# dscripka/openWakeWord

Measured on AMD Instinct MI355X. Metric: real-time audio frames/sec (80 ms frame, 3 wakewords), whole job; real-time streams = value/12.5, higher is better.
Workload: dtype f32 as 3xf16 split MFMA, fp32 accumulate; 1 GPU; 131072 concurrent 16 kHz streams per GPU x 3 heads (alexa,hey_mycroft,hey_jarvis), 80 ms frames, BASELINE configs[3] per-GPU shard; streams_per_gpu=131072, frame_samples=1280, collective=none, gather=none, rccl_ranks=0, pcm_distribution=Gaussian, RMS 3000, pcm=resident in HBM, kernels=mfma_rr_f16x3, graph=False, vad=off, weights=synthetic seed 1234, step_blocks=1

## Files before the change

### openwakeword_amd/csrc/owwhip.hip

```cpp
#include <hip/hip_runtime.h>

#include <algorithm>
#include <cmath>
#include <cstdio>
#include <cstdlib>
#include <cstring>
#include <ctime>
#include <exception>
#include <mutex>
#include <new>
#include <unordered_map>
#include <dlfcn.h>
#include <string>
#include <vector>

#include "owwhip.h"
#include "owwhip_pack.h"
#include "owwhip_ingest.h"
#include "owwhip_mem.h"
#include "owwhip_masked_host.h"
#include "owwhip_bank_host.h"
#include "owwhip_verifier_host.h"
#include "owwhip_state_host.h"
#include "owwhip_kernels.h"
// ... 186 lines not shown
        bool busy = false;
    } slot[2];
    struct EventBuf {
        DevBuf<oww_event> d_rec; DevBuf<int> d_count; DevBuf<float> d_snap;
        DevBuf<int16_t> d_asnap;
        PinnedBuf<oww_event> h_rec; PinnedBuf<int> h_count;
    };
    int evt_cap = 0, evt_rows = 0;
    DevBuf<float> d_evt_thr; float evt_bank_thr = 0.5f;
    DevBuf<int> d_evblock; int evt_blocks = 0;
    EventBuf evt_sync, evt_slot[2];
    const EventBuf* evt_cur = nullptr;
    int aud_ring = 0, aud_evt = 0;
    DevBuf<int16_t> d_aring;
    DevBuf<uint32_t> d_acount;
    DevBuf<int16_t> d_aout; DevBuf<int> d_aids; DevBuf<uint32_t> d_acnt;

    uint64_t n_submit = 0, n_collect = 0;
    DevBuf<float> d_featinit, d_dbg;
    DevBuf<long long> d_prof;
    int prof_block = -1;
    DevBuf<uint32_t> d_nfeat, d_npred, d_nvad;
    DevBuf<float> d_vadring, d_vadin; float vad_threshold = 0.f;
    bool vad = false;
    const float *d_vad_hann = nullptr, *d_vad_encw = nullptr, *d_vad_encb = nullptr, *d_vad_lstmw = nullptr, *d_vad_lstmb = nullptr, *d_vad_wd = nullptr;
    float vad_bd = 0.f, vad_gain = 50.f;
    DevBuf<float> d_vadx, d_vadhc, d_vadlast;
    DevBuf<int16_t> d_tail, d_pcm;
    DevBuf<int16_t> d_long;
    DevBuf<float> d_callmax;
    PinnedBuf<int> h_range;
    int* d_range = nullptr;
    DevBuf<char> d_rs;
    std::vector<float> rs_taps;
    struct Ingest {
        bool ready = false, mixed = false;
        owi::Table tab;
        DevBuf<float> d_taps;
        DevBuf<int16_t> d_hist;
        DevBuf<int16_t> d_out;
        DevBuf<char> d_in;
        DevBuf<uint8_t> d_on;
        DevBuf<IngestClass> d_table;
        DevBuf<uint32_t> d_cls;
        DevBuf<int> d_newcls;
    } ing;
    DevBuf<uint8_t> d_on;
    DevBuf<int> d_lists; PinnedBuf<int> h_lists[2]; owm::Event lists_ev[2]; unsigned lists_turn = 0;
    int k_last = 1;
    float hx_absmax[20] = {};
    std::vector<int16_t> cal_user;
    int small_wgs = kSmallLaunchWgs, small_wgs_heads = kSmallLaunchWgs;
    int resident_b = -1, resident_b_wgs = kResidentBWgs;
    float hx_selftest_err = 0.f, hx_selftest_ref = 0.f, hx_selftest_score_err = 0.f;
    bool fuse = false;
    DevBuf<float> d_verw, d_verb, d_verthr; DevBuf<int> d_verT;
    int ver_stride = 0, n_verifiers = 0;
    std::vector<int> ver_T;
    bool post_in_heads = false;
    DevBuf<float> d_save;
    DevBuf<int> d_ids;
    DevBuf<int> d_patience;
    DevBuf<float> d_threshold;
    int debounce_frames = 0;
    void* comm = nullptr; int comm_rank = 0, comm_world = 1;
    bool timing = false;
    std::vector<EventRec> ev;
    size_t ev_used = 0;
    double t_ms[OWW_N_KERNEL_CLASSES] = {};
    int64_t t_n[OWW_N_KERNEL_CLASSES] = {};
    bool want_graph = false;
    hipGraph_t graph = nullptr;
    hipGraphExec_t graph_exec = nullptr;
    struct BankHead {
        bool live = false;
        int T = 0, hidden = 0, has_ln = 0, ht = 4, patience = 0;
        float threshold = NAN;
        DevBuf<float> d_img;
        size_t w1_bytes = 0;
        owh::BankHeadDev dev{};
    };
    int bank_K = 0, bank_cap = 0;
    std::vector<BankHead> bank;
    std::vector<int> bank_sub;
    DevBuf<int> d_bank_sub, d_bank_idx;
    DevBuf<float> d_bank_raw, d_bank_scores, d_bank_ring;
    DevBuf<uint32_t> d_bank_npred;
    DevBuf<owh::BankHeadDev> d_bank_heads; DevBuf<int> d_bank_pat; DevBuf<float> d_bank_thr;
    DevBuf<owh::BankTile> d_bank_tiles; DevBuf<int> d_bank_entries;
    owb::Route bank_rt;
    int vpool_cap = 0;
    int vpool_stride = 0;
    std::vector<int> vpool_T;
    DevBuf<float> d_vpool_w, d_vpool_b;
    std::vector<int> vasg_fix, vasg_bank;
    std::vector<float> vthr_fix, vthr_bank;
    long long vasg_n = 0;
    std::vector<float> ver_thr;
    DevBuf<SvEntry> d_svlist; int sv_n = 0;
    DevBuf<unsigned long long> d_sv_eval;
    bool st_ready = false;
    std::vector<ows::FlatSection> st_flat;
    std::vector<ows::GroupSection> st_group;
    bool st_levels[4] = {};
    DevBuf<ows::FlatSection> d_st_flat;
    uint32_t st_record_words = 0, st_flat_quads = 0;
// ... 72 lines not shown
        p.xout = h->d_xA; p.dbg = dbg ? h->d_dbg : nullptr; p.dbg_stride = DBG_FLOATS;
        Timed t(h, 1);
        hipLaunchKernelGGL(stageA_kernel<MFMA>, dim3(n_active), dim3(CfgA::NT), CfgA::LDS_BYTES, st, p);
    }
    auto fill = [&](StageParams& p, const float* xin, float* xout, int first_layer, int sb, int sd) {
        p.xin = xin; p.xout = xout; p.hist_b = h->d_state[sb]; p.hist_d = h->d_state[sd];
        for (int i = 0; i < 4; ++i) {
            p.w[i] = h->d_conv[first_layer + i]; p.scale[i] = h->d_scale[first_layer + i];
            p.shift[i] = h->d_shift[first_layer + i]; p.dbg_off[i] = dbg_off[first_layer + i];
        }
        p.dbg = dbg ? h->d_dbg : nullptr; p.dbg_stride = DBG_FLOATS;
        p.prof = h->d_prof ? h->d_prof + (first_layer / 4) * 256 : nullptr;
        p.prof_block = h->prof_block;
    };
    {
        StageParams p{}; fill(p, h->d_xA, h->d_xB, 3, 2, 3);
        Timed t(h, 2);
        hipLaunchKernelGGL((stage_kernel<CfgB, MFMA, false>), dim3((n_active + CfgB::B - 1) / CfgB::B), dim3(CfgB::NT), CfgB::LDS_BYTES, st, p);
    }
    {
        StageParams p{}; fill(p, h->d_xB, h->d_xC, 7, 4, 5);
        Timed t(h, 3);
        hipLaunchKernelGGL((stage_kernel<CfgC, MFMA, false>), dim3((n_active + CfgC::B - 1) / CfgC::B), dim3(CfgC::NT), CfgC::LDS_BYTES, st, p);
    }
    {
        StageParams p{}; fill(p, h->d_xC, h->d_xD, 11, 6, 7);
        Timed t(h, 4);
        hipLaunchKernelGGL((stage_kernel<CfgD, MFMA, false>), dim3((n_active + CfgD::B - 1) / CfgD::B), dim3(CfgD::NT), CfgD::LDS_BYTES, st, p);
    }
    {
        StageParams p{}; fill(p, h->d_xD, nullptr, 15, 8, 9);
        p.hist19 = h->d_state[10]; p.w19 = h->d_conv[19]; p.feat = h->d_feat; p.emb = h->d_emb; p.nfeat = h->d_nfeat; p.TR = h->TR;
        p.dbg_off[4] = dbg_off[19];
        Timed t(h, 5);
        hipLaunchKernelGGL((stage_kernel<CfgE, MFMA, true>), dim3((n_active + CfgE::B - 1) / CfgE::B), dim3(CfgE::NT), CfgE::LDS_BYTES, st, p);
    }
    HIPCHK(hipGetLastError());
    return 0;
}

template <class CR, class CH, int WG, bool LAST, bool DBG, bool HX>
void launch_rstage(oww_ctx* h, const owr::RStageParams& p, int cls) {
    hipStream_t st = h->stream;
    Timed t(h, cls);
    const int nwg = (p.n_groups + WG - 1) / WG;
    if constexpr (HX && !DBG && std::is_same<CH, owh::HB>::value) {
        const bool resident = p.glist == nullptr && p.n_groups > 0 && (h->resident_b < 0 ? p.n_groups >= kResidentBMinGroups : h->resident_b != 0);
        if (resident) {
            const int grid = std::max(1, std::min(h->resident_b_wgs, (p.n_groups + owh::RES_B_WG - 1) / owh::RES_B_WG));
            hipLaunchKernelGGL((owh::hstage_kernel<CH, LAST, false, owh::RES_B_WG, 1>), dim3(grid), dim3(64 * owh::RES_B_WG), owh::RES_B_LDS_BYTES, st, p);
            return;
        }
    }
    if (HX && !DBG && nwg <= h->small_wgs) hipLaunchKernelGGL((owh::hstage_kernel<CH, LAST, false, WG, 3>), dim3(nwg), dim3(64 * WG), 0, st, p);
    else if (HX) hipLaunchKernelGGL((owh::hstage_kernel<CH, LAST, DBG, WG>), dim3(nwg), dim3(64 * WG), 0, st, p);
    else hipLaunchKernelGGL((owr::rstage_kernel<CR, LAST, DBG>), dim3((p.n_groups + 3) / 4), dim3(256), 0, st, p);
}

template <bool DBG, bool HX>
int run_cnn_rr(oww_ctx* h, const StepArgs& a, int n_active, int mel_stride, int mel_off) {
    using namespace owr;
    hipStream_t st = h->stream;
    int off = 0, dbg_off[20];
    for (int l = 0; l < 20; ++l) { dbg_off[l] = off; off += kLayerOut[l][0] * kLayerOut[l][1] * kLayerOut[l][2]; }
    {
        RAParams p{};
        p.mel = a.mel ? a.mel : h->d_mel; p.mel_stride = mel_stride; p.mel_off = mel_off;
        p.hist_mel = h->d_state[0]; p.hist2 = h->d_state[1];
        p.w0 = h->d_conv[0]; p.w1 = h->d_conv[1]; p.w2 = h->d_conv[2];
        for (int i = 0; i < 3; ++i) { p.scale[i] = h->d_scale[i]; p.shift[i] = h->d_shift[i]; p.dbg_off[i] = dbg_off[i]; }
        p.xout = h->d_xA; p.n_streams = n_active; p.S = h->Spad;
        p.dbg = DBG ? h->d_dbg : nullptr; p.dbg_stride = DBG_FLOATS;
        for (int i = 0; i < 3; ++i) { p.clampv[i] = -0.4f * ldexpf(1.f, h->hx_e[i]); p.dbg_mul[i] = ldexpf(1.f, -h->hx_e[i]); }
        p.xmul = ldexpf(1.f, h->hx_xexp[0]);
        p.range_flag = HX ? h->d_range : nullptr;
        p.stream_on = a.on;
        const int grid = std::min((n_active + 3) / 4, 768);
        Timed t(h, 1);
        if (HX && a.fused_pcm) {
            owf::MelAParams q{};
            q.a = p; q.a.mel = nullptr; q.a.n_streams = h->S;
            q.pcm = a.fused_pcm; q.tail = h->d_tail; q.nfeat = h->d_nfeat; q.hann = h->d_hann; q.mel_start = h->d_mstart; q.mel_taps = h->d_taps; q.mel_off = h->d_meloff; q.mel_dst = h->d_meldst;
            q.mel_out = h->cfg.debug_layers ? h->d_mel : nullptr;
            const int per_cu = std::max(1, std::min(12 / owf::FA_WG, 163840 / owf::FA_LDS_BYTES));
            const int g2 = std::max(1, std::min((q.a.n_streams + owf::FA_WG - 1) / owf::FA_WG, 256 * per_cu));
            hipLaunchKernelGGL(owf::hmelA_kernel<DBG>, dim3(g2), dim3(64 * owf::FA_WG), owf::FA_LDS_BYTES, st, q);
        }
        else if (HX) hipLaunchKernelGGL(owh::hstageA_kernel<DBG>, dim3(std::min((n_active + 3) / 4, 256 * OWH_WPS_A)), dim3(256), 0, st, p);
        else hipLaunchKernelGGL(rstageA_kernel<DBG>, dim3(grid), dim3(256), 0, st, p);
    }
    auto fill = [&](const float* xin, float* xout, int first_layer, int sb, int sd, int spt) {
        RStageParams p{};
        p.xin = xin; p.xout = xout; p.hist_b = h->d_state[sb]; p.hist_d = h->d_state[sd];
        for (int i = 0; i < 4; ++i) {
            p.w[i] = h->d_conv[first_layer + i]; p.scale[i] = h->d_scale[first_layer + i];
            p.shift[i] = h->d_shift[first_layer + i]; p.dbg_off[i] = dbg_off[first_layer + i];
            p.clampv[i] = -0.4f * ldexpf(1.f, h->hx_e[first_layer + i]); p.dbg_mul[i] = ldexpf(1.f, -h->hx_e[first_layer + i]);
        }
        p.dbg_mul[4] = ldexpf(1.f, -h->hx_e[19]);
        p.xmul = ldexpf(1.f, h->hx_xexp[first_layer / 4 + 1]);
        p.emb_mul = ldexpf(1.f, -h->hx_e[19]);
        p.n_groups = (n_active + spt - 1) / spt; p.S = h->Spad;
        p.dbg = DBG ? h->d_dbg : nullptr; p.dbg_stride = DBG_FLOATS;
        p.range_flag = HX ? h->d_range : nullptr;
        p.stream_on = a.on;
        if (HX && a.lists) {
// ... 1370 lines not shown
    if (absmax) memcpy(absmax, h->hx_absmax, sizeof h->hx_absmax);
    if (exps) { for (int l = 0; l < 20; ++l) exps[l] = h->hx_e[l]; exps[20] = h->hx_efeat; }
    if (n_probe_streams) *n_probe_streams = CAL_NP + (int32_t)(h->cal_user.size() / ((size_t)CAL_T * OWW_CHUNK));
    if (selftest) { selftest[0] = h->hx_selftest_err; selftest[1] = h->hx_selftest_ref; selftest[2] = h->hx_selftest_score_err; }
    return OWW_OK;
    OWW_GUARD_END
}

int oww_n_labels(const oww_ctx* h) { return h ? h->NL : 0; }

int oww_commit(oww_ctx* h) {
    OWW_GUARD_BEGIN
    if (!h) return fail(OWW_EINVAL, "null handle");
    if (h->committed) return fail(OWW_ESTATE, "already committed");
    if (h->mel_blob.empty() || h->emb_blob.empty()) return fail(OWW_ESTATE, "mel and embedding weights must be loaded before commit");
    HIPCHK(hipSetDevice(h->cfg.device));
    h->feature_ring = h->cfg.feature_ring;
    if (int rc = build_nets(*h, h->NL, h->TR, h->generic_hmax)) return rc;
    if (h->evt_rows > h->TR)
        return fail(OWW_EINVAL, "oww_events_configure: feature_rows = %d exceeds the handle's feature ring (%d rows)", h->evt_rows, h->TR);
    if (int rc = owa::commit_check(h->aud_evt, h->evt_cap)) return rc;
    CommitClock clk(h->hx ? "f16-split" : "family");
    HxCalib cal;
    if (h->hx) {
        if (int rc = calibrate_hx(h, cal)) return rc;
        h->probe_emb = cal.ref_emb; h->probe_nb = cal.nb;
        clk.lap("calibration (total)");
        if (getenv("OWW_DEBUG_CALIB"))
            for (int l = 0; l < 20; ++l) fprintf(stderr, "calib layer %2d: max|a| %-12.5g e_in %4d e_out %4d\n", l, h->hx_absmax[l], h->hx_ein[l], h->hx_e[l]);
    }
    HostBuf hb;
    WeightOff off;
    HeadGroups hg;
    h->no_wide_heads = getenv("OWW_NO_WIDE_HEADS") != nullptr;
    if (int rc = pack_mel_tables(*h, hb, off)) return rc;
    if (int rc = pack_cnn(*h, hb, off)) return rc;
    pack_net_arrays(*h, hb, off);
    if (int rc = pack_head_groups(*h, hg, hb, off)) return rc;
    h->groups.clear();
    for (const HeadGroup& g : hg.groups) h->groups.push_back(FastGroup{g});
    h->generic_nets = hg.generic_nets; h->rnn_nets = hg.rnn_nets;
    h->vad = !h->vad_blob.empty();
    if (int rc = pack_vad(*h, hb, off, h->vad_gain, h->vad_bd)) return rc;
    clk.lap("weight packing (host)");
    if (int rc = bind_weights(h, hb, off)) return rc;
    if (int rc = alloc_range_flag(h)) return rc;
    clk.lap("weight upload");
    if (int rc = alloc_state(h)) return rc;
    h->fuse = h->hx && !getenv("OWW_NO_FUSE");
    if (const char* e = getenv("OWW_SMALL_WGS")) h->small_wgs = atoi(e);
    if (const char* e = getenv("OWW_SMALL_WGS_HEADS")) h->small_wgs_heads = atoi(e);
    if (const char* e = getenv("OWW_RESIDENT_B")) h->resident_b = strcmp(e, "auto") == 0 ? -1 : (atoi(e) != 0 ? 1 : 0);
    if (const char* e = getenv("OWW_RESIDENT_B_WGS")) h->resident_b_wgs = std::max(1, atoi(e));
    if (const char* e = getenv("OWW_GENERIC_SPW")) { const int v = atoi(e); h->generic_spw = v == 4 || v == 16 ? v : 0; }
    h->post_in_heads = h->fuse && h->groups.size() == 1 && h->groups[0].ht == 4 && h->generic_nets.empty() && h->rnn_nets.empty() && h->NL > 0;
    if (int rc = set_kernel_lds(h)) return rc;
    clk.lap("state allocation");
    if (int rc = derive_reset_state(h, cal, clk)) return rc;
    if (h->bank_K > 0) if (int rc = alloc_bank(h)) return rc;
    if (h->vpool_cap > 0) if (int rc = alloc_verifiers(h)) return rc;
    if (audio_on(h)) if (int rc = alloc_audio(h)) return rc;
    if (events_on(h)) if (int rc = alloc_events(h)) return rc;
    h->committed = true;
    return OWW_OK;
    OWW_GUARD_END
}

int oww_reset(oww_ctx* h, const int32_t* stream_ids, int32_t n, const float* init_features) {
    OWW_GUARD_BEGIN
    if (!h || !h->committed) return fail(OWW_ESTATE, "oww_reset: handle not committed");
    HIPCHK(hipSetDevice(h->cfg.device));
    const float* d_init = nullptr;
    if (init_features) {
        HIPCHK(copy_async(h->d_featinit, init_features, (size_t)h->TR * 96 * sizeof(float), hipMemcpyHostToDevice, h->stream));
        d_init = h->d_featinit;
    }
    if (!stream_ids) {
        if (int rc = do_reset(h, nullptr, h->Spad, d_init)) return rc;
    } else {
        if (n < 1) return OWW_OK;
        for (int i = 0; i < n; ++i)
            if (stream_ids[i] < 0 || stream_ids[i] >= h->S) return fail(OWW_EINVAL, "oww_reset: stream id %d out of range", stream_ids[i]);
        if (int rc = upload_ids(h, stream_ids, n)) return rc;
        if (int rc = do_reset(h, h->d_ids, n, d_init)) return rc;
    }
    if (h->ing.ready && h->ing.tab.Hpad_max) {
        hipLaunchKernelGGL(ingest_hist_reset_kernel, dim3(stream_ids ? n : h->S), dim3(64), 0, h->stream, h->ing.d_hist, h->ing.tab.Hpad_max,
                           stream_ids ? h->d_ids : nullptr, stream_ids ? n : h->S);
        HIPCHK(hipGetLastError());
    }
    if (audio_on(h)) if (int rc = audio_reset(h, stream_ids ? (const int*)h->d_ids : nullptr, n)) return rc;
    std::vector<int> slots;
    if (h->bank_K > 0) {
        if (!stream_ids) for (int i = 0; i < h->S * h->bank_K; ++i) slots.push_back(i);
        else for (int i = 0; i < n; ++i) for (int k = 0; k < h->bank_K; ++k) slots.push_back(stream_ids[i] * h->bank_K + k);
        if (int rc = bank_clear(h, slots)) return rc;
    }
    HIPCHK(hipStreamSynchronize(h->stream));
    return OWW_OK;
    OWW_GUARD_END
}

int oww_set_postproc(oww_ctx* h, const int32_t* patience, const float* threshold, int32_t debounce_frames) {
    OWW_GUARD_BEGIN
    if (!h || !h->committed) return fail(OWW_ESTATE, "oww_set_postproc: handle not committed");
    HIPCHK(hipSetDevice(h->cfg.device));
// ... 1574 lines not shown
```

### openwakeword_amd/csrc/owwhip_hx.h

```cpp
#pragma once
#include <type_traits>
#include <utility>
#include "owwhip_bank_host.h"
#include "owwhip_layout.h"
#include "owwhip_rr.h"

namespace owh {

using owr::f32x4;
typedef _Float16 f16x8 __attribute__((ext_vector_type(8)));

constexpr float WUNSCALE = 1.0f / 256.0f;

__device__ __forceinline__ float act1(float x, float cl) {
    return fmaxf(fmaxf(0.2f * x, x), cl);
}
template <bool ACT, bool HALF>
__device__ __forceinline__ f32x4 act_t(const f32x4 v, float cl) {
    if (!ACT) return HALF ? f32x4{v[0], v[1], 0.f, 0.f} : v;
    if (HALF) return f32x4{act1(v[0], cl), act1(v[1], cl), 0.f, 0.f};
    return f32x4{act1(v[0], cl), act1(v[1], cl), act1(v[2], cl), act1(v[3], cl)};
}
template <bool HALF>
__device__ __forceinline__ void pin_t(f32x4& v) {
// ... 337 lines not shown
                        const float l = dpp_shr_zero<SH>(accs[0][t][e]);
                        acc[t][e] = unpaired<F>(I[e] + ((MASKS && first) ? 0.f : l));
                    }
                }
            }
#pragma unroll
            for (int ks = 0; ks < KSI; ++ks) {
                f16x8 ah, al;
                if constexpr (AP) {
                    const int g = ti * KSI + ks;
                    const int ntap = ks + 1 < KSI ? tap : (ti == 0 ? 2 : 1), nks = ks + 1 < KSI ? ks + 1 : 0;
                    apipe_step(ap[g & 1], ap[(g + 1) & 1], cur, g + 1 < 3 * KSI ? (ntap * KSI + nks) * 2 : -1, lane);
                    ah = ap[g & 1].h; al = ap[g & 1].l;
                } else {
                    ah = lds_h(cur, (tap * KSI + ks) * 2 + 0, lane);
                    al = lds_h(cur, (tap * KSI + ks) * 2 + 1, lane);
                }
                if (REM2 && ks == KSI - 1) {
#pragma unroll
                    for (int t = 0; t < NT; ++t) acc[t] = OWH_MFMA(ah, in[t][ks].l, acc[t]);
#pragma unroll
                    for (int t = 0; t < NT; ++t) acc[t] = OWH_MFMA(al, in[t][ks].h, acc[t]);
                    continue;
                }
#pragma unroll
                for (int t = 0; t < NT; ++t) acc[t] = OWH_MFMA(ah, in[t][ks].h, acc[t]);
#pragma unroll
                for (int t = 0; t < NT; ++t) acc[t] = OWH_MFMA(ah, in[t][ks].l, acc[t]);
#pragma unroll
                for (int t = 0; t < NT; ++t) acc[t] = OWH_MFMA(al, in[t][ks].h, acc[t]);
            }
#pragma unroll
            for (int t = 0; t < NT; ++t) {
                if (ti < 2) accs[ti][t] = acc[t];
                else {
#pragma unroll
                    for (int e = 0; e < 4; ++e) {
                        if (HOUT && oct == NCTO - 1 && e >= 2) { res[t][e] = 0.f; continue; }
                        const float hh = dpp_shl_zero<SH>(accs[1][t][e]);
                        res[t][e] = acc[t][e] + ((MASKS && last) ? 0.f : hh);
                    }
                }
            }
        }
        if (oct == 0) {
#pragma unroll
            for (int t = 0; t < NT; ++t) nan_guard(bad, res[t][0]);
        }
#pragma unroll
        for (int t = 0; t < NT; ++t) {
            if (HOUT && oct == NCTO - 1) { out[t][oct] = act_t<BN, true>(res[t], cl); pin_t<true>(out[t][oct]); }
            else { out[t][oct] = act_t<BN, false>(res[t], cl); pin_t<false>(out[t][oct]); }
        }
        ring_end<NS, NBLK, NCTO, NEXT_NBLK, WG>(oct);
    }
}

template <int KSI, int NT, int F, int NPR>
__device__ __forceinline__ void merge_mel_rems(const Op (&in)[NT][KSI], Op (&M)[NT][(3 * NPR + 3) / 4]) {
    typedef unsigned u32x4 __attribute__((ext_vector_type(4)));
    static_assert(kInterleave || F == 16, "the operand shift relies on the zero fill at the stream edges");
    constexpr int SH = 16 / F, NMK = (3 * NPR + 3) / 4;
#pragma unroll
    for (int t = 0; t < NT; ++t) {
        const u32x4 sh = __builtin_bit_cast(u32x4, in[t][KSI - 1].h), sl = __builtin_bit_cast(u32x4, in[t][KSI - 1].l);
        unsigned h[NMK * 4], l[NMK * 4];
#pragma unroll
        for (int i = 0; i < NMK * 4; ++i) {
            const int tap = i / NPR, v = i % NPR;
            if (i >= 3 * NPR) { h[i] = 0u; l[i] = 0u; }
            else if (tap == 0) { h[i] = __builtin_amdgcn_update_dpp(0, sh[v], 0x110 + SH, 0xf, 0xf, true); l[i] = __builtin_amdgcn_update_dpp(0, sl[v], 0x110 + SH, 0xf, 0xf, true); }
            else if (tap == 2) { h[i] = __builtin_amdgcn_update_dpp(0, sh[v], 0x100 + SH, 0xf, 0xf, true); l[i] = __builtin_amdgcn_update_dpp(0, sl[v], 0x100 + SH, 0xf, 0xf, true); }
            else { h[i] = sh[v]; l[i] = sl[v]; }
        }
#pragma unroll
        for (int mk = 0; mk < NMK; ++mk) {
            M[t][mk].h = __builtin_bit_cast(f16x8, u32x4{h[4 * mk], h[4 * mk + 1], h[4 * mk + 2], h[4 * mk + 3]});
            M[t][mk].l = __builtin_bit_cast(f16x8, u32x4{l[4 * mk], l[4 * mk + 1], l[4 * mk + 2], l[4 * mk + 3]});
            pin_op(M[t][mk]);
        }
    }
}
template <int KSI, int NMK, int NCTO, int NT, int F, bool BN, int CH0, int NEXT_NBLK, int WG = OWH_WG, bool HOUT = false, int NS = 2, bool AP = false>
__device__ __forceinline__ void conv_mel_hxm(const Op (&in)[NT][KSI], const Op (&M)[NT][NMK], f32x4 (&out)[NT][NCTO], const WRing<NS>& ring,
                                             const float* __restrict__ w, const float* __restrict__ w_next,
                                             const float* __restrict__ init, float cl, int wave, int lane,
                                             lanemask_t& bad) {
    using namespace owr;
    const int j = lane >> 4;
    constexpr int SH = 16 / F, KSF = KSI - 1;
    constexpr int NBLK = (3 * KSF + NMK) * 2;
#pragma unroll
    for (int oct = 0; oct < NCTO; ++oct) {
        const float* cur = ring_begin<NS, CH0, NBLK, NCTO, NEXT_NBLK, WG>(ring, oct, w, w_next, wave, lane);
        f32x4 res[NT], accs[2][NT];
        APair ap[2];
        if constexpr (AP) ap[0] = apair_load(cur, 0, lane);
        int g = 0;
#pragma unroll
        for (int ti = 0; ti < 3; ++ti) {
            const int tap = ti == 0 ? 0 : (ti == 1 ? 2 : 1);
            f32x4 acc[NT];
            f32x4 I = {0.f, 0.f, 0.f, 0.f};
            if (ti == 2) I = acc_init(BN ? init : nullptr, oct, j);
#pragma unroll
            for (int t = 0; t < NT; ++t) {
// ... 264 lines not shown
#ifndef OWH_HIST_LDS
#define OWH_HIST_LDS 1
#endif
#ifndef OWH_HIST_LDS_C
#define OWH_HIST_LDS_C 0
#endif
#ifndef OWH_SPRIO_B
#define OWH_SPRIO_B 1111
#endif
#ifndef OWH_SPRIO_RB
#define OWH_SPRIO_RB 1223
#endif
#ifndef OWH_RES_HIST_EARLY
#define OWH_RES_HIST_EARLY 0
#endif
#ifndef OWH_SPRIO_C
#define OWH_SPRIO_C 3210
#endif
#ifndef OWH_SPRIO_D
#define OWH_SPRIO_D 3210
#endif
#ifndef OWH_SPRIO_E
#define OWH_SPRIO_E 1111
#endif
template <int CODE, int LAYER> __device__ __forceinline__ void sprio() {
    constexpr int div = LAYER == 0 ? 1000 : LAYER == 1 ? 100 : LAYER == 2 ? 10 : 1;
    if constexpr (CODE != 0 && LAYER >= 0) __builtin_amdgcn_s_setprio((CODE / div) % 10);
    if constexpr (CODE != 0 && LAYER < 0) __builtin_amdgcn_s_setprio(0);
}
template <int NBLK>
__device__ __forceinline__ void issue_hist(const float* __restrict__ gsrc, float* ldst, int lane) {
    const float* base = owr::uniform_ptr(gsrc);
#pragma unroll
    for (int i = 0; i < NBLK; ++i)
        __builtin_amdgcn_global_load_lds((const __attribute__((address_space(1))) void*)(base + i * 256 + lane * 4),
                                         (__attribute__((address_space(3))) void*)(ldst + i * 256), 16, 0, 0);
}
template <int NCT, bool HALF>
__device__ __forceinline__ void load_tile_lds(f32x4 (&t)[NCT], const float* base, int lane) {
#pragma unroll
    for (int ct = 0; ct < NCT; ++ct)
#pragma unroll
        for (int e = 0; e < 4; ++e) {
            if (HALF && ct == NCT - 1 && e >= 2) t[ct][e] = 0.f;
            else t[ct][e] = base[(ct * 4 + e) * 64 + lane];
        }
}

constexpr int RES_B_WG = 12, RES_B_LDS_BYTES = 126 * 1024;
template <bool RES> __device__ __forceinline__ float* res_lds(float* ring_slot0) {
    if constexpr (RES) { extern __shared__ __attribute__((aligned(16))) float res_dyn[]; return res_dyn; }
    else return ring_slot0;
}
template <class C, bool LAST, bool DBG, int WG = OWH_WG, int NS = 2>
__global__ __launch_bounds__(64 * WG, (DBG || NS > 3 || NS == 1 ? 1 : (NS == 3 && C::WPS > 2 ? 2 : C::WPS))) void hstage_kernel(owr::RStageParams p) {
    using namespace owr;
    constexpr int NCTI = C::NCTI, NCT = C::NCT, R = C::RP, F = C::F;
    static_assert(!LAST || C::NPASS == 1, "the last stage runs in one pass");
    static_assert(NS == 2 || C::NPASS == 1 || (4 * NCT) % NS == 0, "multi-pass stages need a ring phase that returns to 0 after each pass");
    static_assert(NS >= 1 && NS <= 5 && NS - 1 <= NCT, "the chunks in flight at a layer boundary belong to at most the next layer");
    constexpr bool RES = NS == 1;
    static_assert(!RES || (!LAST && !DBG && C::NPASS == 1), "resident weights: one pass, no debug dumps, not the last stage");
    constexpr int KSA = (NCTI + 1) / 2, KS = (NCT + 1) / 2;
    constexpr int NBA = 3 * KSA * 2, NB = 3 * KS * 2;
    using TK = TimeK<NCT, C::HOUT>;
    constexpr bool MERGE = OWH_KMERGE && (NCT % 2 == 1) && !LAST && (C::HOUT || OWH_KMERGE_B);
    constexpr int NBT = MERGE ? TK::NBLK : NB;
    constexpr bool PIPE = OWH_PIPE != 0;
    constexpr int APCFG = NCT == 3 ? OWH_APIPE_B : NCT == 5 ? OWH_APIPE_C : LAST ? OWH_APIPE_E : OWH_APIPE_D;
    constexpr bool APM = (APCFG & 1) != 0, APT = (APCFG & 2) != 0;
    constexpr int SPCODE = NS == 1 ? OWH_SPRIO_RB : NCT == 3 ? OWH_SPRIO_B : NCT == 5 ? OWH_SPRIO_C : LAST ? OWH_SPRIO_E : OWH_SPRIO_D;
    constexpr bool REM2 = OWH_REM2 && NCT % 2 == 1 && !C::HOUT && !LAST && !(OWH_KMERGE && OWH_KMERGE_B) && !(OWH_KMERGE_MEL && OWH_KMERGE_MEL2B);
    constexpr bool MMA2 = OWH_KMERGE_MEL && OWH_KMERGE_MEL2 && kInterleave && !C::HIN && NCTI % 2 == 1 && NCTI >= 3 && C::WPS == 2;
    constexpr bool MMA = (OWH_KMERGE_MEL && kInterleave && C::HIN && NCTI % 2 == 1 && NCTI >= 3) || MMA2;
    constexpr int NPRA = MMA2 ? 2 : 1, NMKA = (3 * NPRA + 3) / 4;
    constexpr bool MMC2 = OWH_KMERGE_MEL && OWH_KMERGE_MEL2B && !C::HOUT && NCT % 2 == 1 && NCT >= 3 && !LAST;
    constexpr bool MMC = (OWH_KMERGE_MEL && kInterleave && C::HOUT && NCT % 2 == 1 && NCT >= 3) || MMC2;
    constexpr int NPRC = MMC2 ? 2 : 1, NMKC = (3 * NPRC + 3) / 4;
    constexpr int NBAM = MMA ? (3 * (KSA - 1) + NMKA) * 2 : NBA, NBCM = MMC ? (3 * (KS - 1) + NMKC) * 2 : NB;
    constexpr int NBMAX = (NBAM > NBT ? NBAM : NBT) > (NBCM > (LAST ? NB : 0) ? NBCM : (LAST ? NB : 0)) ? (NBAM > NBT ? NBAM : NBT) : (NBCM > (LAST ? NB : 0) ? NBCM : (LAST ? NB : 0));
    constexpr int WBS = NBMAX * 256;
    constexpr bool HLDS = OWH_HIST_LDS && !RES && !LAST && C::NPASS == 1 && (C::SPT == 1 || (C::SPT == 2 && OWH_HIST_LDS_C));
    constexpr int HROW = NCT * 4 * 64;
    const int lane0 = threadIdx.x & 63;
    const int wave = __builtin_amdgcn_readfirstlane(threadIdx.x >> 6);
    int g = blockIdx.x * WG + wave;
    __shared__ __attribute__((aligned(16))) float wbuf[RES ? 4 : WBS];
    __shared__ __attribute__((aligned(16))) float wbuf1[RES ? 4 : WBS];
    __shared__ __attribute__((aligned(16))) float wbuf2[NS >= 3 ? WBS : 4];
    __shared__ __attribute__((aligned(16))) float wbuf3[NS >= 4 ? WBS : 4];
    __shared__ __attribute__((aligned(16))) float wbuf4[NS >= 5 ? WBS : 4];
    constexpr int RES_OFF_B = NCT * NBAM * 256, RES_OFF_C = RES_OFF_B + NCT * NBT * 256, RES_OFF_D = RES_OFF_C + NCT * NBCM * 256;
    static_assert(!RES || (RES_OFF_D + NCT * NBT * 256) * 4 == RES_B_LDS_BYTES, "launch_rstage sizes the dynamic LDS with RES_B_LDS_BYTES");
    float* const rw = res_lds<RES>(wbuf);
    const WRing<NS> ring{{rw, RES ? rw + RES_OFF_B : wbuf1, RES ? rw + RES_OFF_C : wbuf2, RES ? rw + RES_OFF_D : wbuf3, wbuf4}};
    __shared__ __attribute__((aligned(16))) float sbn[4][NCT * 16];
    __shared__ __attribute__((aligned(16))) float hlds[HLDS ? WG * 2 * HROW : 4];
    float* const hl = hlds + (HLDS ? wave * 2 * HROW : 0);
    __shared__ int res_next;
    const bool active = RES || g < p.n_groups;
    int g_end = 0;
    if constexpr (RES) {
        const int nwg = gridDim.x, per = p.n_groups / nwg, rem = p.n_groups % nwg, b = blockIdx.x;
        const int g_lo = b * per + min(b, rem);
        g_end = g_lo + per + (b < rem ? 1 : 0);
        if (threadIdx.x == 0) res_next = g_lo;
        constexpr int off4[5] = {0, RES_OFF_B / 4, RES_OFF_C / 4, RES_OFF_D / 4, RES_B_LDS_BYTES / 16};
        constexpr int NT = 64 * WG, MAXU = (off4[2] - off4[1] + NT - 1) / NT;
        static_assert(off4[1] <= MAXU * NT && off4[3] - off4[2] <= MAXU * NT && off4[4] - off4[3] <= MAXU * NT, "layer b's array is the largest");
        f32x4 t[4][MAXU];
#pragma unroll
        for (int l = 0; l < 4; ++l)
#pragma unroll
            for (int u = 0; u < MAXU; ++u) {
                const int i = threadIdx.x + u * NT;
                if (i < off4[l + 1] - off4[l]) t[l][u] = reinterpret_cast<const f32x4*>(p.w[l])[i];
            }
#pragma unroll
        for (int l = 0; l < 4; ++l)
#pragma unroll
            for (int u = 0; u < MAXU; ++u) {
                const int i = threadIdx.x + u * NT;
                if (i < off4[l + 1] - off4[l]) reinterpret_cast<f32x4*>(rw)[off4[l] + i] = t[l][u];
            }
    } else {
    if (!active) g = p.n_groups - 1;
    if (p.glist) g = p.glist[g];
    else g += p.g_base;
    }
    lanemask_t bad = 0;
    if constexpr (!RES) {
    ring_issue<NS, NBAM, WG>(p.w[0], wbuf, wave, lane0);
    if (NS >= 3) ring_issue<NS, NBAM, WG>(p.w[0] + (size_t)NBAM * 256, wbuf1, wave, lane0);
    if (NS >= 4) ring_issue<NS, NBAM, WG>(p.w[0] + (size_t)2 * NBAM * 256, wbuf2, wave, lane0);
    if (NS >= 5) ring_issue<NS, NBAM, WG>(p.w[0] + (size_t)3 * NBAM * 256, wbuf3, wave, lane0);
    }
    for (int i = threadIdx.x; i < 4 * NCT * 16; i += 64 * WG) {
        const int l = i / (NCT * 16), c = i % (NCT * 16);
        sbn[l][c] = p.shift[l][c];
    }
    if constexpr (RES) __syncthreads();
    for (;;) {
    int lane_z = 0;
    if constexpr (RES) asm volatile("" : "+v"(lane_z));
    const int lane = RES ? ((lane0 + lane_z) & 63) : lane0;
    if constexpr (RES) {
        int k = 0;
        if (lane0 == 0) k = __hip_atomic_fetch_add(&res_next, 1, __ATOMIC_RELAXED, __HIP_MEMORY_SCOPE_WORKGROUP);
        g = __builtin_amdgcn_readfirstlane(k);
        if (g >= g_end) break;
        g += p.g_base;
        bad = 0;
    }
    const int s_first = g * C::SPT;
    const bool lane_on = active && (p.stream_on == nullptr || p.stream_on[min(s_first + tile_stream<F>(lane & 15), p.S - 1)] != 0);
    float* hb = p.hist_b + (size_t)g * C::HIST_FLOATS;
    float* hd = p.hist_d + (size_t)g * C::HIST_FLOATS;
    if (HLDS) issue_hist<2 * NCT>(hb, hl, lane);

#pragma unroll
    for (int pass = 0; pass < C::NPASS; ++pass) {
    f32x4 Y[R][NCT];
    Op Xo[R][KSA];
#pragma unroll
    for (int r = 0; r < R; ++r) {
        f32x4 X[NCTI];
        load_tile_h<NCTI, C::HIN>(X, p.xin + ((size_t)price_alias<(OWH_PRICE_HANDOVER & 2) != 0 && C::CIN == 24>(g) * C::R + pass * R + r) * (NCTI * 4 * 64), lane);
        to_ops<NCTI, C::HIN>(X, Xo[r]);
    }
    constexpr bool HEARLY = RES && OWH_RES_HIST_EARLY != 0 && !MERGE;
    f32x4 E0[HEARLY ? NCT : 1], E1[HEARLY ? NCT : 1];
    if constexpr (HEARLY) { load_tile_h<NCT, C::HOUT>(E0, hb, lane); load_tile_h<NCT, C::HOUT>(E1, hb + NCT * 4 * 64, lane); }
    if (!RES && pass == 0) chunk_sync();
    sprio<SPCODE, 0>();

    if constexpr (MMA) {
        Op Mx[R][NMKA];
        merge_mel_rems<KSA, R, F, NPRA>(Xo, Mx);
        conv_mel_hxm<KSA, NMKA, NCT, R, F, true, 0, NBT, WG, C::HOUT, NS, APM>(Xo, Mx, Y, ring, p.w[0], p.w[1], sbn[0], p.clampv[0], wave, lane, bad);
    } else
    conv_mel_hx<KSA, NCT, R, F, true, 0, NBT, WG, C::HOUT, false, NS, APM>(Xo, Y, ring, p.w[0], p.w[1], sbn[0], p.clampv[0], wave, lane, bad);
    if (DBG && p.dbg && active) {
#pragma unroll
        for (int r = 0; r < R; ++r) dump_tile_ht<NCT, F, C::C>(Y[r], p.dbg, p.dbg_stride, p.dbg_off[0], s_first, pass * R + r, p.S, lane, p.dbg_mul[0]);
    }
    Op Ao[R][KS], H0[KS], H1[KS];
    sprio<SPCODE, 1>();
    if constexpr (MERGE) {
        Op AoF[R][TK::KSF], H0F[TK::KSF], H1F[TK::KSF], M[R][TK::NMK];
        RemPairs rem[R + 2];
        {
            f32x4 T0[NCT], T1[NCT];
            if (HLDS) { load_tile_lds<NCT, C::HOUT>(T0, hl, lane); load_tile_lds<NCT, C::HOUT>(T1, hl + HROW, lane); }
            else { load_tile_h<NCT, C::HOUT>(T0, hb, lane); load_tile_h<NCT, C::HOUT>(T1, hb + NCT * 4 * 64, lane); }
            to_ops_time<NCT, C::HOUT>(T0, H0F, rem[0]);
            to_ops_time<NCT, C::HOUT>(T1, H1F, rem[1]);
        }
        if (HLDS) { asm volatile("s_waitcnt lgkmcnt(0)" ::: "memory"); issue_hist<2 * NCT>(hd, hl, lane); }
        if (lane_on) {
            store_tile_h<NCT, C::HOUT>(Y[R - 2], hb, lane);
            store_tile_h<NCT, C::HOUT>(Y[R - 1], hb + NCT * 4 * 64, lane);
        }
#pragma unroll
        for (int r = 0; r < R; ++r) to_ops_time<NCT, C::HOUT>(Y[r], AoF[r], rem[2 + r]);
        merge_rems<R, TK::NPR, TK::NMK>(rem, M);
        __builtin_amdgcn_sched_barrier(0);
        conv_time_hxm<TK::KSF, TK::NMK, NCT, R, true, NCT, NBCM, WG, C::HOUT, NS, APT>(H0F, H1F, AoF, M, Y, ring, p.w[1], p.w[2], sbn[1], p.clampv[1], wave, lane, bad);
    } else {
    if constexpr (HEARLY) { to_ops<NCT, C::HOUT, REM2>(E0, H0); to_ops<NCT, C::HOUT, REM2>(E1, H1); }
    else {
        f32x4 T0[NCT], T1[NCT];
        if (HLDS) { load_tile_lds<NCT, C::HOUT>(T0, hl, lane); load_tile_lds<NCT, C::HOUT>(T1, hl + HROW, lane); }
        else { load_tile_h<NCT, C::HOUT>(T0, hb, lane); load_tile_h<NCT, C::HOUT>(T1, hb + NCT * 4 * 64, lane); }
        to_ops<NCT, C::HOUT, REM2>(T0, H0);
        to_ops<NCT, C::HOUT, REM2>(T1, H1);
    }
    if (HLDS) { asm volatile("s_waitcnt lgkmcnt(0)" ::: "memory"); issue_hist<2 * NCT>(hd, hl, lane); }
    if (lane_on) {
        store_tile_h<NCT, C::HOUT>(Y[R - 2], hb, lane);
        store_tile_h<NCT, C::HOUT>(Y[R - 1], hb + NCT * 4 * 64, lane);
    }
#pragma unroll
    for (int r = 0; r < R; ++r) to_ops<NCT, C::HOUT, REM2>(Y[r], Ao[r]);
    __builtin_amdgcn_sched_barrier(0);
    conv_time_hx<KS, NCT, R, true, NCT, NBCM, WG, true, C::HOUT, PIPE, REM2, NS, APT>(H0, H1, Ao, Y, ring, p.w[1], p.w[2], sbn[1], p.clampv[1], wave, lane, bad);
    }
    if (DBG && p.dbg && active) {
#pragma unroll
        for (int r = 0; r < R; ++r) dump_tile_ht<NCT, F, C::C>(Y[r], p.dbg, p.dbg_stride, p.dbg_off[1], s_first, pass * R + r, p.S, lane, p.dbg_mul[1]);
    }
#pragma unroll
    for (int r = 0; r < R; ++r) to_ops<NCT, C::HOUT, REM2>(Y[r], Ao[r]);
    __builtin_amdgcn_sched_barrier(0);
    if constexpr (HEARLY) { load_tile_h<NCT, C::HOUT>(E0, hd, lane); load_tile_h<NCT, C::HOUT>(E1, hd + NCT * 4 * 64, lane); }
    sprio<SPCODE, 2>();
    if constexpr (MMC) {
        Op Mc[R][NMKC];
        merge_mel_rems<KS, R, F, NPRC>(Ao, Mc);
        conv_mel_hxm<KS, NMKC, NCT, R, F, true, 2 * NCT, NBT, WG, C::HOUT, NS, APM>(Ao, Mc, Y, ring, p.w[2], p.w[3], sbn[2], p.clampv[2], wave, lane, bad);
    } else
    conv_mel_hx<KS, NCT, R, F, true, 2 * NCT, NBT, WG, C::HOUT, REM2, NS, APM>(Ao, Y, ring, p.w[2], p.w[3], sbn[2], p.clampv[2], wave, lane, bad);
    if (DBG && p.dbg && active) {
#pragma unroll
        for (int r = 0; r < R; ++r) dump_tile_ht<NCT, F, C::C>(Y[r], p.dbg, p.dbg_stride, p.dbg_off[2], s_first, pass * R + r, p.S, lane, p.dbg_mul[2]);
    }
    sprio<SPCODE, 3>();
    if constexpr (MERGE) {
        Op AoF[R][TK::KSF], H0F[TK::KSF], H1F[TK::KSF], M[R][TK::NMK];
        RemPairs rem[R + 2];
        {
            f32x4 T0[NCT], T1[NCT];
            if (HLDS) { load_tile_lds<NCT, C::HOUT>(T0, hl, lane); load_tile_lds<NCT, C::HOUT>(T1, hl + HROW, lane); }
            else { load_tile_h<NCT, C::HOUT>(T0, hd, lane); load_tile_h<NCT, C::HOUT>(T1, hd + NCT * 4 * 64, lane); }
            to_ops_time<NCT, C::HOUT>(T0, H0F, rem[0]);
            to_ops_time<NCT, C::HOUT>(T1, H1F, rem[1]);
        }
        if (lane_on) {
            store_tile_h<NCT, C::HOUT>(Y[R - 2], hd, lane);
            store_tile_h<NCT, C::HOUT>(Y[R - 1], hd + NCT * 4 * 64, lane);
        }
#pragma unroll
        for (int r = 0; r < R; ++r) to_ops_time<NCT, C::HOUT>(Y[r], AoF[r], rem[2 + r]);
        merge_rems<R, TK::NPR, TK::NMK>(rem, M);
        __builtin_amdgcn_sched_barrier(0);
        conv_time_hxm<TK::KSF, TK::NMK, NCT, R, true, 3 * NCT, (C::NPASS > 1 ? NBAM : 0), WG, C::HOUT, NS, APT>(H0F, H1F, AoF, M, Y, ring, p.w[3], p.w[0], sbn[3], p.clampv[3], wave, lane, bad);
    } else {
    if constexpr (HEARLY) { to_ops<NCT, C::HOUT, REM2>(E0, H0); to_ops<NCT, C::HOUT, REM2>(E1, H1); }
    else {
        f32x4 T0[NCT], T1[NCT];
        if (HLDS) { load_tile_lds<NCT, C::HOUT>(T0, hl, lane); load_tile_lds<NCT, C::HOUT>(T1, hl + HROW, lane); }
        else { load_tile_h<NCT, C::HOUT>(T0, hd, lane); load_tile_h<NCT, C::HOUT>(T1, hd + NCT * 4 * 64, lane); }
        to_ops<NCT, C::HOUT, REM2>(T0, H0);
        to_ops<NCT, C::HOUT, REM2>(T1, H1);
    }
    if (lane_on) {
        store_tile_h<NCT, C::HOUT>(Y[R - 2], hd, lane);
        store_tile_h<NCT, C::HOUT>(Y[R - 1], hd + NCT * 4 * 64, lane);
    }
#pragma unroll
    for (int r = 0; r < R; ++r) to_ops<NCT, C::HOUT, REM2>(Y[r], Ao[r]);
    __builtin_amdgcn_sched_barrier(0);
    conv_time_hx<KS, NCT, R, true, 3 * NCT, (LAST ? NB : (C::NPASS > 1 ? NBAM : 0)), WG, true, C::HOUT, PIPE, REM2, NS, APT>(H0, H1, Ao, Y, ring, p.w[3], LAST ? p.w19 : p.w[0], sbn[3], p.clampv[3], wave, lane, bad);
    }
    if (DBG && p.dbg && active) {
#pragma unroll
        for (int r = 0; r < R; ++r) dump_tile_ht<NCT, F, C::C>(Y[r], p.dbg, p.dbg_stride, p.dbg_off[3], s_first, pass * R + r, p.S, lane, p.dbg_mul[3]);
    }

    sprio<SPCODE, -1>();
    if (!LAST && lane_on) {
        constexpr int FO = C::FO, RO = C::RO;
        constexpr int SPTN = 16 / FO;
        const int pos = lane & 15, j = lane >> 4;
// ... 1246 lines not shown
```

Baseline: 24.03 million frames/s.

## Add mel-major retiled 1x3 conv path for the last CNN stage

Adds a new conv_mel_hx_mm routine for the last stage's 1x3 mel convolutions. It swaps the operand halves with DPP lane permutes so each MFMA covers mel-major tiles, then splits taps into separately accumulated partial sums and swaps the results back afterwards. The aim is to cut wasted or redundant MFMA work and dependency chains in the mel convolution, at the cost of extra DPP shuffles. A new kernel template flag selects the path, and it is on by default through retile_e=1, with an OWW_RETILE_E override. The new launch branch also runs ahead of the usual NS choice and uses a ring depth of 2, or 3 for small launches.

```diff
diff --git a/openwakeword_amd/csrc/owwhip.hip b/openwakeword_amd/csrc/owwhip.hip
--- a/openwakeword_amd/csrc/owwhip.hip
+++ b/openwakeword_amd/csrc/owwhip.hip
@@ -262,6 +262,7 @@
     std::vector<int16_t> cal_user;
     int small_wgs = kSmallLaunchWgs, small_wgs_heads = kSmallLaunchWgs;
     int resident_b = -1, resident_b_wgs = kResidentBWgs;
+    int retile_e = 1;
     float hx_selftest_err = 0.f, hx_selftest_ref = 0.f, hx_selftest_score_err = 0.f;
     bool fuse = false;
     DevBuf<float> d_verw, d_verb, d_verthr; DevBuf<int> d_verT;
@@ -440,6 +441,13 @@
             return;
         }
     }
+    if constexpr (HX && LAST) {
+        if (h->retile_e != 0) {
+            if (!DBG && nwg <= h->small_wgs) hipLaunchKernelGGL((owh::hstage_kernel<CH, true, false, WG, 3, true>), dim3(nwg), dim3(64 * WG), 0, st, p);
+            else hipLaunchKernelGGL((owh::hstage_kernel<CH, true, DBG, WG, 2, true>), dim3(nwg), dim3(64 * WG), 0, st, p);
+            return;
+        }
+    }
     if (HX && !DBG && nwg <= h->small_wgs) hipLaunchKernelGGL((owh::hstage_kernel<CH, LAST, false, WG, 3>), dim3(nwg), dim3(64 * WG), 0, st, p);
     else if (HX) hipLaunchKernelGGL((owh::hstage_kernel<CH, LAST, DBG, WG>), dim3(nwg), dim3(64 * WG), 0, st, p);
     else hipLaunchKernelGGL((owr::rstage_kernel<CR, LAST, DBG>), dim3((p.n_groups + 3) / 4), dim3(256), 0, st, p);
@@ -1916,6 +1924,7 @@
     if (const char* e = getenv("OWW_SMALL_WGS_HEADS")) h->small_wgs_heads = atoi(e);
     if (const char* e = getenv("OWW_RESIDENT_B")) h->resident_b = strcmp(e, "auto") == 0 ? -1 : (atoi(e) != 0 ? 1 : 0);
     if (const char* e = getenv("OWW_RESIDENT_B_WGS")) h->resident_b_wgs = std::max(1, atoi(e));
+    if (const char* e = getenv("OWW_RETILE_E")) h->retile_e = strcmp(e, "auto") == 0 ? 1 : (atoi(e) != 0 ? 1 : 0);
     if (const char* e = getenv("OWW_GENERIC_SPW")) { const int v = atoi(e); h->generic_spw = v == 4 || v == 16 ? v : 0; }
     h->post_in_heads = h->fuse && h->groups.size() == 1 && h->groups[0].ht == 4 && h->generic_nets.empty() && h->rnn_nets.empty() && h->NL > 0;
     if (int rc = set_kernel_lds(h)) return rc;
diff --git a/openwakeword_amd/csrc/owwhip_hx.h b/openwakeword_amd/csrc/owwhip_hx.h
--- a/openwakeword_amd/csrc/owwhip_hx.h
+++ b/openwakeword_amd/csrc/owwhip_hx.h
@@ -413,6 +413,100 @@
             if (HOUT && oct == NCTO - 1) { out[t][oct] = act_t<BN, true>(res[t], cl); pin_t<true>(out[t][oct]); }
             else { out[t][oct] = act_t<BN, false>(res[t], cl); pin_t<false>(out[t][oct]); }
         }
+        ring_end<NS, NBLK, NCTO, NEXT_NBLK, WG>(oct);
+    }
+}
+
+__device__ __forceinline__ void mel_major_swap(unsigned& a, unsigned& b) {
+    const unsigned na = (unsigned)__builtin_amdgcn_update_dpp((int)a, (int)b, 0x118, 0xf, 0xc, false);
+    const unsigned nb = (unsigned)__builtin_amdgcn_update_dpp((int)b, (int)a, 0x108, 0xf, 0x3, false);
+    a = na; b = nb;
+}
+__device__ __forceinline__ void mel_major_swap(f16x8& a, f16x8& b) {
+    typedef unsigned u32x4 __attribute__((ext_vector_type(4)));
+    u32x4 x = __builtin_bit_cast(u32x4, a), y = __builtin_bit_cast(u32x4, b);
+    unsigned xs[4] = {x[0], x[1], x[2], x[3]}, ys[4] = {y[0], y[1], y[2], y[3]};
+#pragma unroll
+    for (int v = 0; v < 4; ++v) mel_major_swap(xs[v], ys[v]);
+    a = __builtin_bit_cast(f16x8, u32x4{xs[0], xs[1], xs[2], xs[3]});
+    b = __builtin_bit_cast(f16x8, u32x4{ys[0], ys[1], ys[2], ys[3]});
+}
+template <int KSI, int NCTO, bool BN, int CH0, int NEXT_NBLK, int WG = OWH_WG, int NS = 2, bool AP = false>
+__device__ __forceinline__ void conv_mel_hx_mm(Op (&in)[2][KSI], f32x4 (&out)[2][NCTO], const WRing<NS>& ring,
+                                               const float* __restrict__ w, const float* __restrict__ w_next,
+                                               const float* __restrict__ init, float cl, int wave, int lane,
+                                               lanemask_t& bad) {
+    using namespace owr;
+    static_assert(kInterleave, "mel-major tiles regroup the interleaved position order");
+    const int j = lane >> 4;
+    constexpr int NBLK = 3 * KSI * 2;
+#pragma unroll
+    for (int ks = 0; ks < KSI; ++ks) {
+        mel_major_swap(in[0][ks].h, in[1][ks].h);
+        mel_major_swap(in[0][ks].l, in[1][ks].l);
+        pin_op(in[0][ks]); pin_op(in[1][ks]);
+    }
+#pragma unroll
+    for (int oct = 0; oct < NCTO; ++oct) {
+        const float* cur = ring_begin<NS, CH0, NBLK, NCTO, NEXT_NBLK, WG>(ring, oct, w, w_next, wave, lane);
+        APair ap[2], aq[2];
+        if constexpr (AP) { ap[0] = apair_load(cur, 0, lane); aq[0] = apair_load(cur, 2 * KSI * 2, lane); }
+        f32x4 s0 = {0.f, 0.f, 0.f, 0.f}, s2 = {0.f, 0.f, 0.f, 0.f};
+#pragma unroll
+        for (int ks = 0; ks < KSI; ++ks) {
+            f16x8 a0h, a0l, a2h, a2l;
+            if constexpr (AP) {
+                apair_pin(ap[ks & 1]); apair_pin(aq[ks & 1]);
+                if (ks + 1 < KSI) { ap[(ks + 1) & 1] = apair_load(cur, (ks + 1) * 2, lane); aq[(ks + 1) & 1] = apair_load(cur, (2 * KSI + ks + 1) * 2, lane); }
+                else ap[(ks + 1) & 1] = apair_load(cur, KSI * 2, lane);
+                __builtin_amdgcn_sched_barrier(0);
+                a0h = ap[ks & 1].h; a0l = ap[ks & 1].l; a2h = aq[ks & 1].h; a2l = aq[ks & 1].l;
+            } else {
+                a0h = lds_h(cur, ks * 2 + 0, lane); a0l = lds_h(cur, ks * 2 + 1, lane);
+                a2h = lds_h(cur, (2 * KSI + ks) * 2 + 0, lane); a2l = lds_h(cur, (2 * KSI + ks) * 2 + 1, lane);
+            }
+            s0 = OWH_MFMA(a0h, in[0][ks].h, s0);
+            s2 = OWH_MFMA(a2h, in[1][ks].h, s2);
+            s0 = OWH_MFMA(a0h, in[0][ks].l, s0);
+            s2 = OWH_MFMA(a2h, in[1][ks].l, s2);
+            s0 = OWH_MFMA(a0l, in[0][ks].h, s0);
+            s2 = OWH_MFMA(a2l, in[1][ks].h, s2);
+        }
+        const f32x4 I = acc_init(BN ? init : nullptr, oct, j);
+        f32x4 acc[2];
+#pragma unroll
+        for (int e = 0; e < 4; ++e) { acc[0][e] = I[e]; acc[1][e] = I[e] + s0[e]; }
+#pragma unroll
+        for (int ks = 0; ks < KSI; ++ks) {
+            f16x8 ah, al;
+            if constexpr (AP) {
+                const int g = KSI + ks;
+                apipe_step(ap[g & 1], ap[(g + 1) & 1], cur, ks + 1 < KSI ? (KSI + ks + 1) * 2 : -1, lane);
+                ah = ap[g & 1].h; al = ap[g & 1].l;
+            } else {
+                ah = lds_h(cur, (KSI + ks) * 2 + 0, lane);
+                al = lds_h(cur, (KSI + ks) * 2 + 1, lane);
+            }
+#pragma unroll
+            for (int t = 0; t < 2; ++t) acc[t] = OWH_MFMA(ah, in[t][ks].h, acc[t]);
+#pragma unroll
+            for (int t = 0; t < 2; ++t) acc[t] = OWH_MFMA(ah, in[t][ks].l, acc[t]);
+#pragma unroll
+            for (int t = 0; t < 2; ++t) acc[t] = OWH_MFMA(al, in[t][ks].h, acc[t]);
+        }
+        f32x4 res[2];
+#pragma unroll
+        for (int e = 0; e < 4; ++e) {
+            unsigned u = __builtin_bit_cast(unsigned, acc[0][e] + s2[e]), v = __builtin_bit_cast(unsigned, acc[1][e] + 0.f);
+            mel_major_swap(u, v);
+            res[0][e] = __builtin_bit_cast(float, u); res[1][e] = __builtin_bit_cast(float, v);
+        }
+        if (oct == 0) {
+#pragma unroll
+            for (int t = 0; t < 2; ++t) nan_guard(bad, res[t][0]);
+        }
+#pragma unroll
+        for (int t = 0; t < 2; ++t) { out[t][oct] = act_t<BN, false>(res[t], cl); pin_t<false>(out[t][oct]); }
         ring_end<NS, NBLK, NCTO, NEXT_NBLK, WG>(oct);
     }
 }
@@ -783,10 +877,11 @@
     if constexpr (RES) { extern __shared__ __attribute__((aligned(16))) float res_dyn[]; return res_dyn; }
     else return ring_slot0;
 }
-template <class C, bool LAST, bool DBG, int WG = OWH_WG, int NS = 2>
+template <class C, bool LAST, bool DBG, int WG = OWH_WG, int NS = 2, bool RT = false>
 __global__ __launch_bounds__(64 * WG, (DBG || NS > 3 || NS == 1 ? 1 : (NS == 3 && C::WPS > 2 ? 2 : C::WPS))) void hstage_kernel(owr::RStageParams p) {
     using namespace owr;
     constexpr int NCTI = C::NCTI, NCT = C::NCT, R = C::RP, F = C::F;
+    static_assert(!RT || (LAST && F == 2 && R == 2 && kInterleave && !C::HIN && !C::HOUT), "mel-major 1x3 layers: two rows of 2 mel positions x 8 streams, full channel tiles");
     static_assert(!LAST || C::NPASS == 1, "the last stage runs in one pass");
     static_assert(NS == 2 || C::NPASS == 1 || (4 * NCT) % NS == 0, "multi-pass stages need a ring phase that returns to 0 after each pass");
     static_assert(NS >= 1 && NS <= 5 && NS - 1 <= NCT, "the chunks in flight at a layer boundary belong to at most the next layer");
@@ -868,7 +963,9 @@
     }
     for (int i = threadIdx.x; i < 4 * NCT * 16; i += 64 * WG) {
         const int l = i / (NCT * 16), c = i % (NCT * 16);
-        sbn[l][c] = p.shift[l][c];
+        float v = p.shift[l][c];
+        if (RT && (l & 1) == 0) v += 0.f;
+        sbn[l][c] = v;
     }
     if constexpr (RES) __syncthreads();
     for (;;) {
@@ -909,7 +1006,9 @@
         Op Mx[R][NMKA];
         merge_mel_rems<KSA, R, F, NPRA>(Xo, Mx);
         conv_mel_hxm<KSA, NMKA, NCT, R, F, true, 0, NBT, WG, C::HOUT, NS, APM>(Xo, Mx, Y, ring, p.w[0], p.w[1], sbn[0], p.clampv[0], wave, lane, bad);
-    } else
+    } else if constexpr (RT)
+    conv_mel_hx_mm<KSA, NCT, true, 0, NBT, WG, NS, APM>(Xo, Y, ring, p.w[0], p.w[1], sbn[0], p.clampv[0], wave, lane, bad);
+    else
     conv_mel_hx<KSA, NCT, R, F, true, 0, NBT, WG, C::HOUT, false, NS, APM>(Xo, Y, ring, p.w[0], p.w[1], sbn[0], p.clampv[0], wave, lane, bad);
     if (DBG && p.dbg && active) {
 #pragma unroll
@@ -969,7 +1068,9 @@
         Op Mc[R][NMKC];
         merge_mel_rems<KS, R, F, NPRC>(Ao, Mc);
         conv_mel_hxm<KS, NMKC, NCT, R, F, true, 2 * NCT, NBT, WG, C::HOUT, NS, APM>(Ao, Mc, Y, ring, p.w[2], p.w[3], sbn[2], p.clampv[2], wave, lane, bad);
-    } else
+    } else if constexpr (RT)
+    conv_mel_hx_mm<KS, NCT, true, 2 * NCT, NBT, WG, NS, APM>(Ao, Y, ring, p.w[2], p.w[3], sbn[2], p.clampv[2], wave, lane, bad);
+    else
     conv_mel_hx<KS, NCT, R, F, true, 2 * NCT, NBT, WG, C::HOUT, REM2, NS, APM>(Ao, Y, ring, p.w[2], p.w[3], sbn[2], p.clampv[2], wave, lane, bad);
     if (DBG && p.dbg && active) {
 #pragma unroll
```

After: 24.16 million frames/s, median of 6. About the same (+0.5%).
